# pqpeqr/RL-2048-with-Reinforce-and-Actor-Critic

Hardware: NVIDIA B200
Metric: 2048 env-steps/sec (random-legal batched env stepping, 1M packed boards per GPU) (higher is better)
Workload: dtype u64

## Files before the change

rl-2048-with-reinforce-and-actor-critic_b200/csrc/b2048_device.cuh:

```cuda
#pragma once
#include <stdint.h>

#if defined(__CUDACC__)
#define B2_HD __host__ __device__ __forceinline__
#else
#define B2_HD static inline
#endif

namespace b2 {

struct Board {
    uint32_t lo, hi;
};

B2_HD Board make_board(uint64_t b) { return Board{(uint32_t)b, (uint32_t)(b >> 32)}; }
B2_HD uint64_t to_u64(Board b) { return (uint64_t)b.lo | ((uint64_t)b.hi << 32); }

B2_HD uint32_t prmt(uint32_t x, uint32_t y, uint32_t s) {
#if defined(__CUDA_ARCH__)
    uint32_t r;
    asm("prmt.b32 %0, %1, %2, %3;" : "=r"(r) : "r"(x), "r"(y), "r"(s));
    return r;
#else
    uint64_t v = (uint64_t)x | ((uint64_t)y << 32);
// ... 48 lines not shown
    asm("lop3.b32 %0, %1, %2, %3, 0xE4;" : "=r"(r) : "r"(on1), "r"(on0), "r"(mask));
    return r;
#else
    return (on1 & mask) | (on0 & ~mask);
#endif
}

B2_HD uint32_t nz8(uint32_t x) { return (((x & 0x77777777u) + 0x77777777u) | x) & 0x88888888u; }

struct Rand4 {
    uint32_t w0, w1, w2, w3;
};

B2_HD Rand4 philox4x32_10(uint32_t c0, uint32_t c1, uint32_t c2, uint32_t c3, uint32_t k0, uint32_t k1) {
    const uint32_t M0 = 0xD2511F53u, M1 = 0xCD9E8D57u, W0 = 0x9E3779B9u, W1 = 0xBB67AE85u;
#pragma unroll
    for (int r = 0; r < 10; ++r) {
        uint32_t h0 = mulhi(M0, c0), l0 = M0 * c0;
        uint32_t h1 = mulhi(M1, c2), l1 = M1 * c2;
        c0 = h1 ^ c1 ^ k0;
        c1 = l1;
        c2 = h0 ^ c3 ^ k1;
        c3 = l0;
        k0 += W0;
        k1 += W1;
    }
    return Rand4{c0, c1, c2, c3};
}

struct PhiloxKeys {
    uint32_t k0[10], k1[10];
};
B2_HD PhiloxKeys make_keys(uint64_t seed) {
    PhiloxKeys k;
    uint32_t a = (uint32_t)seed, b = (uint32_t)(seed >> 32);
    for (int r = 0; r < 10; ++r) { k.k0[r] = a; k.k1[r] = b; a += 0x9E3779B9u; b += 0xBB67AE85u; }
    return k;
}
B2_HD Rand4 philox_keyed(uint32_t c0, uint32_t c1, uint32_t c2, uint32_t c3, const PhiloxKeys& k) {
    const uint32_t M0 = 0xD2511F53u, M1 = 0xCD9E8D57u;
#pragma unroll
    for (int r = 0; r < 10; ++r) {
        uint64_t p0 = (uint64_t)M0 * c0, p1 = (uint64_t)M1 * c2;
        c0 = (uint32_t)(p1 >> 32) ^ c1 ^ k.k0[r];
        c1 = (uint32_t)p1;
        c2 = (uint32_t)(p0 >> 32) ^ c3 ^ k.k1[r];
        c3 = (uint32_t)p0;
    }
    return Rand4{c0, c1, c2, c3};
}
B2_HD Rand4 stream_keyed(const PhiloxKeys& k, uint64_t gid, uint32_t t, uint32_t domain) {
    return philox_keyed((uint32_t)gid, (uint32_t)(gid >> 32), t, domain, k);
}

B2_HD Rand4 stream(uint64_t seed, uint64_t gid, uint32_t t, uint32_t domain) {
    return philox4x32_10((uint32_t)gid, (uint32_t)(gid >> 32), t, domain, (uint32_t)seed, (uint32_t)(seed >> 32));
}

struct Xform {
    uint32_t st;
    uint32_t sm;
    uint32_t f_lo, f_hi, i_lo, i_hi;
};

B2_HD Xform xform_for(uint32_t a) {
    const uint64_t F_LO = 0x3210260423016240ull, F_HI = 0x7654371567457351ull;
    const uint64_t I_LO = 0x3210735123016240ull, I_HI = 0x7654624067457351ull;
    uint32_t sh = 16u * a;
    Xform x;
    x.st = (a & 1u) ? 0u : 12u;
    x.sm = ((a ^ (a >> 1)) & 1u) ? 4u : 0u;
    x.f_lo = (uint32_t)(F_LO >> sh);
    x.f_hi = (uint32_t)(F_HI >> sh);
    x.i_lo = (uint32_t)(I_LO >> sh);
    x.i_hi = (uint32_t)(I_HI >> sh);
    return x;
}

B2_HD uint32_t blk_transpose(uint32_t x, uint32_t s) {
    return bitsel(0x0F0F0000u, x << s, bitsel(0x0000F0F0u, x >> s, x));
}
B2_HD uint32_t nib_swap(uint32_t x, uint32_t s) {
    return bitsel(0xF0F0F0F0u, x << s, x >> s);
}

B2_HD Board canon_fwd(Board b, const Xform& x) {
    uint32_t lo = nib_swap(blk_transpose(b.lo, x.st), x.sm);
    uint32_t hi = nib_swap(blk_transpose(b.hi, x.st), x.sm);
    return Board{prmt(lo, hi, x.f_lo), prmt(lo, hi, x.f_hi)};
}
B2_HD Board canon_inv(Board b, const Xform& x) {
    uint32_t lo = prmt(b.lo, b.hi, x.i_lo), hi = prmt(b.lo, b.hi, x.i_hi);
    return Board{blk_transpose(nib_swap(lo, x.sm), x.st), blk_transpose(nib_swap(hi, x.sm), x.st)};
}

B2_HD void row_move_left(uint32_t row, uint32_t& out, uint32_t& merge) {
    uint32_t cells[4];
    int n = 0;
#pragma unroll
    for (int c = 0; c < 4; ++c) {
        uint32_t e = (row >> (4 * c)) & 0xFu;
        if (e) cells[n++] = e;
    }
    out = 0;
    merge = 0;
    int i = 0, w = 0, nm = 0;
    while (i < n) {
        if (i + 1 < n && cells[i] == cells[i + 1]) {
            uint32_t e = cells[i] + 1;
            out |= (e > 15u ? 15u : e) << (4 * w);
            merge |= (e > 15u ? 1u : e) << (4 * nm);
            ++nm;
            i += 2;
        } else {
            out |= cells[i] << (4 * w);
            i += 1;
        }
        ++w;
    }
}

struct MoveResult {
    Board board;
    uint32_t merge;
};

template <typename LutL, typename LutM>
B2_HD MoveResult move_board(Board b, uint32_t a, LutL lut_left, LutM lut_merge) {
    Xform x = xform_for(a);
    Board c = canon_fwd(b, x);
    uint32_t i0 = c.lo & 0xFFFFu, i1 = c.lo >> 16, i2 = c.hi & 0xFFFFu, i3 = c.hi >> 16;
    uint32_t r0 = lut_left[i0], r1 = lut_left[i1], r2 = lut_left[i2], r3 = lut_left[i3];
    uint32_t m0 = lut_merge[i0], m1 = lut_merge[i1], m2 = lut_merge[i2], m3 = lut_merge[i3];
    Board moved{r0 | (r1 << 16), r2 | (r3 << 16)};
    MoveResult res;
    res.board = canon_inv(moved, x);
    res.merge = m0 | (m1 << 8) | (m2 << 16) | (m3 << 24);
    return res;
}

struct MergeStats {
    uint32_t n;
    uint32_t sum_log2;
    uint32_t sum;
    uint32_t max_exp;
    bool overflow;
};

B2_HD MergeStats merge_stats(uint32_t m, bool want_sum, bool want_max) {
    MergeStats s;
    uint32_t nzb = nz8(m);
    s.n = (uint32_t)popc(nzb);
    uint32_t is1 = nzb & ~nz8(m ^ 0x11111111u);
    s.overflow = is1 != 0u;
    uint32_t pairs = (m & 0x0F0F0F0Fu) + ((m >> 4) & 0x0F0F0F0Fu);
    pairs = (pairs & 0x00FF00FFu) + ((pairs >> 8) & 0x00FF00FFu);
    s.sum_log2 = (pairs + (pairs >> 16)) & 0xFFFFu;
    s.sum = 0;
    s.max_exp = 0;
    if (s.overflow) s.sum_log2 += 15u * (uint32_t)popc(is1);
    if (want_sum || want_max) {
#pragma unroll
        for (int k = 0; k < 8; ++k) {
            uint32_t e = (m >> (4 * k)) & 0xFu;
            e = (e == 1u) ? 16u : e;
            if (want_sum) s.sum += e ? (1u << e) : 0u;
// ... 84 lines not shown
```

rl-2048-with-reinforce-and-actor-critic_b200/csrc/b2048_env.cu:

```cuda
#include <cuda_runtime.h>

#include <cstdio>
#include <cstdlib>

#include "b2048_internal.h"
#include "b2048_ptx.cuh"
#include "b2048_step_fast.cuh"

namespace b2 {

__global__ void build_lut_kernel(uint16_t* __restrict__ lut_left, uint8_t* __restrict__ lut_merge) {
    uint32_t row = blockIdx.x * blockDim.x + threadIdx.x;
    if (row >= 65536u) return;
    uint32_t out, merge;
    row_move_left(row, out, merge);
    lut_left[row] = (uint16_t)out;
    lut_merge[row] = (uint8_t)merge;
}

__global__ void build_small_tables_kernel(uint8_t* __restrict__ small) {
    static_assert(B2048_SMALL_BYTES == B2048_TABLES_BYTES - B2048_LUT_BYTES, "small table size mismatch");
    const uint32_t tid = threadIdx.x;
    if (tid < 256u) small_table_entry_agg(tid, reinterpret_cast<AggEntry*>(small + B2048_SMALL_AGG_OFF)[tid]);
    if (tid < 4u) small_table_entry_sel(tid, reinterpret_cast<SelEntry*>(small + B2048_SMALL_SEL_OFF)[tid]);
// ... 159 lines not shown
            if (cfg.action_mode == B2048_ACT_BUFFER) io.action = args.action[i];
            if (args.flags_in) io.mask_in = args.flags_in[i];
        }
        if (!lut_ready) {
            mbar_wait(s_u32(&mbar), 0);
            lut_ready = true;
        }
        bool frozen = false;
        Board board_before = io.board;
        if (args.ep_len && valid) frozen = args.ep_len[i] != 0;
        step_one(io, cfg, opt, args.seed, args.gid0 + (uint64_t)i, args.t, lut_left, lut_merge);
        if (valid && frozen) {
            uint32_t m = legal_mask(board_before);
            uint32_t f = args.flags_in ? (uint32_t)args.flags_in[i]
                                       : (m | ((m == 0u && (board_before.lo | board_before.hi) != 0u) ? B2048_F_DONE : 0u));
            args.board_out[i] = to_u64(board_before);
            if (args.action_out) args.action_out[i] = 0;
            if (args.merge_sum) args.merge_sum[i] = 0;
            if (args.reward) args.reward[i] = 0.0f;
            if (args.reward64) args.reward64[i] = 0.0;
            args.flags[i] = (uint8_t)(f & ~B2048_F_CHANGED);
            io.board = board_before;
        } else if (valid) {
            if (args.ep_len && (io.flags & (B2048_F_DONE | B2048_F_TRUNC))) args.ep_len[i] = (int32_t)args.ep_t;
            args.board_out[i] = to_u64(io.board);
            if (args.score) args.score[i] = io.score;
            if (args.step) args.step[i] = io.step;
            if (args.max_exp) args.max_exp[i] = (uint8_t)io.max_exp;
            if (args.action_out) args.action_out[i] = (uint8_t)io.action_played;
            if (args.merge_sum) args.merge_sum[i] = io.merge_sum;
            if (args.reward) args.reward[i] = (float)io.reward;
            if (args.reward64) args.reward64[i] = io.reward;
            args.flags[i] = (uint8_t)io.flags;
        }
        if (args.obs != nullptr && cfg.obs_mode != B2048_OBS_NONE) {
            const int64_t warp_base = base + (tid & ~31);
            if (cfg.obs_mode == B2048_OBS_ONEHOT) store_obs_onehot(args.obs, io.board, warp_base, args.n, lane);
            else store_obs16(args.obs, io.board, warp_base, args.n, lane, cfg.obs_mode, cfg.obs_log2_scale);
        }
    }
}

template <int kAct, bool kTrack, bool kPlain>
__global__ void __launch_bounds__(1024, 1) step_fast_kernel(const __grid_constant__ StepArgs args) {
    extern __shared__ __align__(128) uint8_t smem[];
    __shared__ uint64_t mbar;
    const int tid = threadIdx.x;
    const bool dbg = args.debug_clock != nullptr && tid == 0 && (blockIdx.x == 0 || blockIdx.x == 147);
    long long* dc = dbg ? args.debug_clock + (blockIdx.x == 0 ? 0 : 16) : nullptr;
    int dci = 0;
    if (dbg) { dc[dci++] = (long long)globaltimer(); dc[dci++] = clock64(); }
    pdl_launch_dependents();
    stage_tables<true>(smem, args, &mbar);
    FastTables T;
    T.left = reinterpret_cast<const uint16_t*>(smem);
    T.merge = smem + B2048_LUT_LEFT_BYTES;
    T.agg = reinterpret_cast<const AggEntry*>(smem + B2048_LUT_BYTES + B2048_SMALL_AGG_OFF);
    T.sel = reinterpret_cast<const SelEntry*>(smem + B2048_LUT_BYTES + B2048_SMALL_SEL_OFF);
    T.act = smem + B2048_LUT_BYTES + B2048_SMALL_ACT_OFF;
    pdl_wait();

    const b2048_env_cfg& cfg = args.cfg;
    if constexpr (kPlain) {
        const uint32_t n = (uint32_t)args.n, stride = gridDim.x * 1024u;
        uint32_t i = blockIdx.x * 1024u + (uint32_t)tid;
        uint2 bw_next = make_uint2(0u, 0u);
        uint32_t act_next = 0u, fin_next = 0u, score_next = 0u, step_next = 0u, max_next = 2u;
        auto request = [&](uint32_t k) {
            bw_next = *reinterpret_cast<const uint2*>(args.board_in + k);
            if (kAct == B2048_ACT_BUFFER) act_next = args.action[k];
            else if (kAct != B2048_ACT_RANDOM_ANY) fin_next = args.flags_in[k];
            if (kTrack) { score_next = args.score[k]; step_next = args.step[k]; max_next = args.max_exp[k]; }
        };
        if (i < n) request(i);
        Rand4 rnd = stream_keyed(args.keys, args.gid0 + (uint64_t)i, args.t, B2048_DOM_STEP);
        mbar_wait(s_u32(&mbar), 0);
        for (; i < n; i += stride) {
            FastIO io;
            io.lo = bw_next.x; io.hi = bw_next.y;
            io.score = score_next; io.step = step_next; io.max_exp = max_next;
            io.action = act_next; io.mask_in = fin_next;
            const uint32_t inext = i + stride;
            if (inext < n) request(inext);
            step_fast_rnd<kAct, kTrack, false>(io, cfg, rnd, args.seed, args.gid0 + (uint64_t)i, args.t, T);
            *reinterpret_cast<uint2*>(args.board_out + i) = make_uint2(io.lo, io.hi);
            if (kTrack) { args.score[i] = io.score; args.step[i] = io.step; args.max_exp[i] = (uint8_t)io.max_exp; }
            args.reward[i] = io.reward;
            args.flags[i] = (uint8_t)io.flags;
            if (inext < n) rnd = stream_keyed(args.keys, args.gid0 + (uint64_t)inext, args.t, B2048_DOM_STEP);
        }
        return;
    }
    bool ready = false;
    const int64_t stride = (int64_t)gridDim.x * 1024;
    int64_t i = (int64_t)blockIdx.x * 1024 + tid;
    uint2 bw_next = make_uint2(0u, 0u);
    uint32_t act_next = 0u, fin_next = 0u;
    if (i < args.n) {
        bw_next = *reinterpret_cast<const uint2*>(args.board_in + i);
        if (kAct == B2048_ACT_BUFFER) act_next = args.action[i];
        if (args.flags_in) fin_next = args.flags_in[i];
    }
    for (; i < args.n; i += stride) {
        FastIO io;
        const uint2 bw = bw_next;
        const uint32_t fin = fin_next;
        io.lo = bw.x; io.hi = bw.y;
        io.score = 0u; io.step = 0u; io.max_exp = 2u; io.mask_in = 0u;
        io.action = act_next;
        const int64_t inext = i + stride;
        if (inext < args.n) {
            bw_next = *reinterpret_cast<const uint2*>(args.board_in + inext);
            if (kAct == B2048_ACT_BUFFER) act_next = args.action[inext];
            if (args.flags_in) fin_next = args.flags_in[inext];
        }
        if (kTrack) { io.score = args.score[i]; io.step = args.step[i]; io.max_exp = args.max_exp[i]; }
        if (kAct == B2048_ACT_RANDOM_LEGAL || kAct == B2048_ACT_PRIORITY)
            io.mask_in = args.flags_in ? fin : legal_mask(Board{io.lo, io.hi});
        bool frozen = false;
        if (args.ep_len) frozen = args.ep_len[i] != 0;
        if (!ready) {
            mbar_wait(s_u32(&mbar), 0);
            ready = true;
            if (dbg) dc[dci++] = clock64();
        }
        if (frozen) {
            uint32_t m = legal_mask(Board{io.lo, io.hi});
            uint32_t f = args.flags_in ? fin : (m | ((m == 0u && (io.lo | io.hi) != 0u) ? B2048_F_DONE : 0u));
            *reinterpret_cast<uint2*>(args.board_out + i) = bw;
            if (args.action_out) args.action_out[i] = 0;
            if (args.merge_sum) args.merge_sum[i] = 0;
            args.reward[i] = 0.0f;
            args.flags[i] = (uint8_t)(f & ~B2048_F_CHANGED);
            continue;
        }
        step_fast<kAct, kTrack>(io, cfg, args.keys, args.seed, args.gid0 + (uint64_t)i, args.t, T);
        if (args.ep_len && (io.flags & (B2048_F_DONE | B2048_F_TRUNC))) args.ep_len[i] = (int32_t)args.ep_t;
        *reinterpret_cast<uint2*>(args.board_out + i) = make_uint2(io.lo, io.hi);
        if (kTrack) { args.score[i] = io.score; args.step[i] = io.step; args.max_exp[i] = (uint8_t)io.max_exp; }
        if (args.action_out) args.action_out[i] = (uint8_t)io.action;
        if (args.merge_sum) args.merge_sum[i] = io.merge_sum;
        args.reward[i] = io.reward;
        args.flags[i] = (uint8_t)io.flags;
        if (dbg && dci < 12) dc[dci++] = clock64();
    }
    if (dbg) { const unsigned long long gt = globaltimer(); dc[14] = clock64(); dc[15] = (long long)gt; }
}

template <int kAct, bool kTrack, bool kPlain>
static cudaError_t launch_fast_one(int grid, size_t smem, cudaStream_t s, const StepArgs& a, bool pdl) {
    cudaLaunchConfig_t lc = {};
    lc.gridDim = dim3((unsigned)grid); lc.blockDim = dim3(1024); lc.dynamicSmemBytes = smem; lc.stream = s;
    cudaLaunchAttribute at[1];
    at[0].id = cudaLaunchAttributeProgrammaticStreamSerialization;
    at[0].val.programmaticStreamSerializationAllowed = 1;
    lc.attrs = at; lc.numAttrs = pdl ? 1u : 0u;
    return cudaLaunchKernelEx(&lc, step_fast_kernel<kAct, kTrack, kPlain>, a);
}
template <int kAct>
static cudaError_t launch_fast(bool track, int grid, size_t smem, cudaStream_t s, const StepArgs& a, bool pdl) {
    const bool plain = a.ep_len == nullptr && a.action_out == nullptr && a.merge_sum == nullptr && a.debug_clock == nullptr &&
                       (kAct == B2048_ACT_BUFFER || kAct == B2048_ACT_RANDOM_ANY || a.flags_in != nullptr) &&
                       a.n < ((int64_t)1 << 31) - (int64_t)grid * 1024 &&
                       !cfg_is_shaped(a.cfg);
    if (plain) return track ? launch_fast_one<kAct, true, true>(grid, smem, s, a, pdl) : launch_fast_one<kAct, false, true>(grid, smem, s, a, pdl);
    return track ? launch_fast_one<kAct, true, false>(grid, smem, s, a, pdl) : launch_fast_one<kAct, false, false>(grid, smem, s, a, pdl);
}
// ... 375 lines not shown
```

rl-2048-with-reinforce-and-actor-critic_b200/csrc/b2048_policy_tc.cu:

```cuda
#include <cuda_bf16.h>
#include <cuda_runtime.h>

#include <cstdio>
#include <cstdlib>

#include "b2048_device.cuh"
#include "b2048_internal.h"
#include "b2048_step_fast.cuh"
#include "b2048_tc.cuh"

namespace b2 {

__global__ void __launch_bounds__(256) policy_tc_prepare_kernel(const float* __restrict__ W1, const float* __restrict__ b1,
                                                                 const float* __restrict__ W2, const float* __restrict__ b2,
                                                                 const float* __restrict__ W3, const float* __restrict__ b3,
                                                                 int n_out, uint8_t* __restrict__ img) {
    const int tid = blockIdx.x * blockDim.x + threadIdx.x;
    const int nth = gridDim.x * blockDim.x;
    auto put = [&](size_t off, float v) { *reinterpret_cast<__nv_bfloat16*>(img + off) = __float2bfloat16_rn(v); };
    for (int idx = tid; idx < TC_H * TC_H; idx += nth) {
        int k = idx / TC_H, n = idx - k * TC_H;
        int slab = k >> 6, kc = (k & 63) >> 3, ke = k & 7;
        put((size_t)IMG_W2 + (size_t)slab * 32768 + (size_t)n * 128 + (size_t)((kc ^ (n & 7)) * 16) + ke * 2, W2[idx]);
    }
// ... 338 lines not shown
                        }
                        if (kRollout) args.ro_actions[slice * stride + b] = (uint8_t)a;
                        else args.action[s] = (uint8_t)a;
                    }
                }
                if (kRollout) {
                    const int g = j & 1, ord = ord_of(j, r);
                    wait_steps_through(g, ord - 1);
                    sAct[g * TC_M + row] = (uint8_t)a;
                    __syncwarp();
                    if (lane == 0) mbar_arrive(bar_act0 + 8u * g);
                    if (dbg) args.debug_clock[8 * item + 6] = clock64();
                    if (!prefetch && item + 1 < n_items) {
                        wait_inputs_of(jn, rn);
                        encode_a1(jn, rn);
                    }
                }
                j = jn; r = rn;
                ph ^= 1u;
            }
        } else if (kRollout) {
            {
                const uint4* src = reinterpret_cast<const uint4*>(args.tables + B2048_LUT_BYTES);
                uint4* dst = reinterpret_cast<uint4*>(smem + SM_TBL);
                for (int i = tid - TC_THREADS; i < B2048_SMALL_BYTES / 16; i += TC_ENV_THREADS) dst[i] = src[i];
                bar_sync(1, TC_ENV_THREADS);
            }
            const int grp = (warp - 21) >> 2;
            const uint32_t bar_act = bar_act0 + 8u * grp, bar_step = bar_step0 + 8u * grp;
            FastTables T;
            T.left = reinterpret_cast<const uint16_t*>(args.tables);
            T.merge = args.tables + B2048_LUT_LEFT_BYTES;
            T.agg = reinterpret_cast<const AggEntry*>(smem + SM_TBL + B2048_SMALL_AGG_OFF);
            T.sel = reinterpret_cast<const SelEntry*>(smem + SM_TBL + B2048_SMALL_SEL_OFF);
            T.act = smem + SM_TBL + B2048_SMALL_ACT_OFF;

            struct EnvIn { uint64_t bd; uint32_t score, step, max_exp, fin; int32_t ep; };
            auto load_in = [&](int j, int r) {
                EnvIn e = {0ull, 0u, 0u, 2u, 0u, 0};
                const int64_t s = tile_of(j) * TC_M + row;
                if (s < n_slots) {
                    const int64_t b = args.slot_map ? args.slot_map[s] : s;
                    const int64_t i = slice_of(r) * args.ro_stride + b;
                    e.bd = args.ro_boards[i]; e.fin = args.ro_flags[i];
                    e.score = args.score[b]; e.step = args.step[b]; e.max_exp = args.max_exp[b];
                    if (args.ep_len) e.ep = args.ep_len[b];
                }
                return e;
            };
            const int own_tiles = (n_owned + 1 - grp) >> 1;
            const int n_rounds = n_owned > 0 ? n_items / n_owned : 0;
            int j = grp, r = own_tiles > 0 ? 0 : n_rounds;
            EnvIn cur = r < n_rounds ? load_in(j, r) : EnvIn{0ull, 0u, 0u, 2u, 0u, 0};
            while (r < n_rounds) {
                int jn = j + 2, rn = r;
                if (jn >= n_owned) { jn = grp; ++rn; }
                const int item = r * n_owned + j;
                const int64_t s = tile_of(j) * TC_M + row;
                const int64_t slice = slice_of(r);
                const bool valid = s < n_slots;
                const int64_t b = (valid && args.slot_map) ? args.slot_map[s] : s;
                const uint32_t t_env = args.t0 + (uint32_t)slice + 1u;
                FastIO io;
                io.lo = (uint32_t)cur.bd; io.hi = (uint32_t)(cur.bd >> 32);
                io.score = cur.score; io.step = cur.step; io.max_exp = cur.max_exp; io.mask_in = 0u;
                const uint32_t fin = cur.fin;
                const bool frozen = cur.ep != 0;
                Rand4 rr = Rand4{0u, 0u, 0u, 0u};
                if (valid && !frozen) rr = stream_keyed(args.keys, args.gid0 + (uint64_t)b, t_env, B2048_DOM_STEP);
                EnvIn nxt = cur;
                if (own_tiles > 1 && rn < n_rounds) nxt = load_in(jn, rn);
                mbar_wait(bar_act, ph);
                const bool dbg = args.debug_clock != nullptr && blockIdx.x == 0 && (tid - TC_THREADS) % TC_ENV_GROUP == 0 && item < 8;
                if (dbg) args.debug_clock[8 * item + 7] = clock64();
                if (valid) {
                    const int64_t o = (slice + 1) * args.ro_stride + b;
                    if (frozen) {
                        args.ro_boards[o] = cur.bd;
                        args.ro_rewards[slice * args.ro_stride + b] = 0.0f;
                        io.flags = fin & ~B2048_F_CHANGED;
                        args.ro_flags[o] = (uint8_t)io.flags;
                    } else {
                        io.action = sAct[grp * TC_M + row];
                        step_fast_rnd<B2048_ACT_BUFFER, true, kShaped>(io, args.cfg, rr, args.seed, args.gid0 + (uint64_t)b, t_env, T);
                        if (args.ep_len && (io.flags & (B2048_F_DONE | B2048_F_TRUNC))) {
                            args.ep_len[b] = (int32_t)(slice + 1);
                            cur.ep = (int32_t)(slice + 1);
                        }
                        args.ro_boards[o] = (uint64_t)io.lo | ((uint64_t)io.hi << 32);
                        args.score[b] = io.score; args.step[b] = io.step; args.max_exp[b] = (uint8_t)io.max_exp;
                        args.ro_rewards[slice * args.ro_stride + b] = io.reward;
                        args.ro_flags[o] = (uint8_t)io.flags;
                    }
                }
                if (own_tiles == 1) {
                    nxt.bd = (uint64_t)io.lo | ((uint64_t)io.hi << 32);
                    nxt.score = io.score; nxt.step = io.step; nxt.max_exp = io.max_exp; nxt.fin = io.flags; nxt.ep = cur.ep;
                }
                cur = nxt;
                j = jn; r = rn;
                __threadfence_block();
                __syncwarp();
                if (lane == 0) mbar_arrive(bar_step);
                ph ^= 1u;
            }
        }
    }

    tmem_teardown(warp == 16, tmem_base, 512u);
}

void launch_tc_prepare(const b2048_mlp_desc* mlp, uint8_t* img, cudaStream_t stream) {
    policy_tc_prepare_kernel<<<64, 256, 0, stream>>>(mlp->W[0], mlp->b[0], mlp->W[1], mlp->b[1], mlp->W[2], mlp->b[2],
                                                      mlp->dims[3], img);
}

int ensure_tc_image(b2048_handle* h) {
    if (!h->tc_image) {
        cudaError_t e = cudaMalloc(&h->tc_image, IMG_BYTES);
        if (e != cudaSuccess) return check_cuda(e, "cudaMalloc(tc_image)");
    }
    if (!(h->attrs & ATTR_POLICY_TC)) {
        cudaError_t e = cudaFuncSetAttribute(policy_tc_kernel<false>, cudaFuncAttributeMaxDynamicSharedMemorySize, SM_TOTAL2);
        if (e != cudaSuccess) return check_cuda(e, "cudaFuncSetAttribute(policy_tc_kernel)");
        e = cudaFuncSetAttribute(policy_tc_kernel<true, false>, cudaFuncAttributeMaxDynamicSharedMemorySize, SM_TOTAL_RO);
        if (e != cudaSuccess) return check_cuda(e, "cudaFuncSetAttribute(policy_tc_kernel<rollout>)");
        e = cudaFuncSetAttribute(policy_tc_kernel<true, true>, cudaFuncAttributeMaxDynamicSharedMemorySize, SM_TOTAL_RO);
        if (e != cudaSuccess) return check_cuda(e, "cudaFuncSetAttribute(policy_tc_kernel<rollout, shaped>)");
        h->attrs |= ATTR_POLICY_TC;
    }
    return B2048_OK;
}

static int print_debug_clock(const b2048_handle* h, cudaStream_t stream) {
    long long hbuf[96];
    { int st = debug_clock_read(h, hbuf, 96, stream); if (st != B2048_OK) return st; }
    for (int k = 0; k < 6; ++k)
        fprintf(stderr,
                "[tc clock] item %d: wait_d1+d3 %lld epi1 %lld wait_d2 %lld epi2 %lld | total %lld | to next %lld | io: d3 seen +%lld, "
                "sample %lld | env: actions seen +%lld\n",
                k, hbuf[8 * k + 1] - hbuf[8 * k], hbuf[8 * k + 2] - hbuf[8 * k + 1], hbuf[8 * k + 3] - hbuf[8 * k + 2],
                hbuf[8 * k + 4] - hbuf[8 * k + 3], hbuf[8 * k + 4] - hbuf[8 * k], hbuf[8 * k + 8] - hbuf[8 * k],
                hbuf[8 * k + 5] - hbuf[8 * k], hbuf[8 * k + 6] - hbuf[8 * k + 5], hbuf[8 * k + 7] - hbuf[8 * k]);
    for (int k = 0; k < 4; ++k)
        fprintf(stderr, "[tc clock] item %d: mma: layer 2 starts +%lld, last H2 slab seen +%lld, d3 committed +%lld | sampler waits for d3 from +%lld\n",
                k, hbuf[64 + 4 * k] - hbuf[8 * k], hbuf[64 + 4 * k + 1] - hbuf[8 * k], hbuf[64 + 4 * k + 2] - hbuf[8 * k],
                hbuf[64 + 4 * k + 3] - hbuf[8 * k]);
    for (int k = 0; k < 4; ++k) fprintf(stderr, "[tc clock] item %d: slowest epilogue warp leaves epilogue 2 at +%lld\n", k, hbuf[80 + k] - hbuf[8 * k]);
    return B2048_OK;
}

int launch_policy_tc(b2048_handle* h, const b2048_mlp_desc* mlp, const uint64_t* board, const uint8_t* mask_flags,
                     uint8_t* action, float* probs, float* logits, int64_t n, uint64_t seed, uint64_t gid0, uint32_t t,
                     int greedy, cudaStream_t stream, bool rebuild_image) {
    if (!fixed_tc_net(mlp) || mlp->dims[3] != 4 || h->smem_optin < SM_TOTAL2) return B2048_ERR_UNSUPPORTED;
    { int st = ensure_tc_image(h); if (st != B2048_OK) return st; }
    if (rebuild_image) launch_tc_prepare(mlp, h->tc_image, stream);
    PolicyTcArgs a{};
    a.img = h->tc_image; a.board = board; a.mask_flags = mask_flags; a.action = action; a.probs = probs; a.logits = logits;
    a.n_out = 4; a.n = n; a.keys = make_keys(seed); a.gid0 = gid0; a.t = t; a.greedy = greedy; a.obs_mode = mlp->obs_mode;
    a.obs_scale = mlp->obs_log2_scale; a.seed = seed; a.n_steps = 1; a.ro_stride = n;
    a.debug_clock = debug_clock_begin(h, B2048_DBG_TC_CLOCKS, stream);
    int64_t tiles = (n + TC_M - 1) / TC_M;
    int grid = (int)(tiles < h->num_sms ? tiles : h->num_sms);
    policy_tc_kernel<false><<<grid, TC_THREADS, SM_TOTAL2, stream>>>(a);
    int st = check_cuda(cudaGetLastError(), "policy_tc_kernel launch");
    if (st == B2048_OK && a.debug_clock) st = print_debug_clock(h, stream);
// ... 50 lines not shown
```

rl-2048-with-reinforce-and-actor-critic_b200/csrc/b2048_step_fast.cuh:

```cuda
#pragma once
#include "b2048_step.cuh"

namespace b2 {

struct SelEntry {
    uint32_t f_lo, f_hi, i_lo, i_hi;
    uint32_t st, sm, pad0, pad1;
};
struct AggEntry {
    uint32_t agg;
    uint32_t orm;
};
#define B2048_SMALL_AGG_OFF 0
#define B2048_SMALL_SEL_OFF 2048
#define B2048_SMALL_ACT_OFF (2048 + 128)
#define B2048_SMALL_BYTES (2048 + 128 + 64)

B2_HD void small_table_entry_agg(uint32_t byte, AggEntry& e) {
    e.agg = 0; e.orm = 0;
    for (int k = 0; k < 2; ++k) {
        uint32_t m = (byte >> (4 * k)) & 0xFu;
        if (!m) continue;
        uint32_t ex = m == 1u ? 16u : m;
        e.agg += (1u << ex) + (ex << 20) + (1u << 28);
        e.orm |= 1u << ex;
    }
}
B2_HD void small_table_entry_sel(uint32_t a, SelEntry& s) {
    Xform x = xform_for(a);
    s.f_lo = x.f_lo & 0xFFFFu; s.f_hi = x.f_hi & 0xFFFFu; s.i_lo = x.i_lo & 0xFFFFu; s.i_hi = x.i_hi & 0xFFFFu;
    s.st = x.st; s.sm = x.sm; s.pad0 = 0; s.pad1 = 0;
}
B2_HD uint32_t small_table_entry_act(uint32_t mask, uint32_t j) {
    uint32_t m = mask;
    for (uint32_t q = 0; q < j; ++q) m &= m - 1;
    return m ? (uint32_t)ffs0(m) : 0u;
}

struct FastTables {
    const uint16_t* left;
    const uint8_t* merge;
    const AggEntry* agg;
    const SelEntry* sel;
    const uint8_t* act;
};

struct FastIO {
    uint32_t lo, hi;
    uint32_t score, step, max_exp;
    uint32_t action;
    uint32_t mask_in;
    float reward;
    uint32_t flags;
    int32_t merge_sum;
};

template <int kAct, bool kTrack, bool kShaped = true>
B2_HD void step_fast_rnd(FastIO& io, const b2048_env_cfg& cfg, const Rand4& rnd, uint64_t seed, uint64_t gid, uint32_t t,
                         const FastTables& T) {

    uint32_t a;
    if (kAct == B2048_ACT_BUFFER) a = io.action & 3u;
    else if (kAct == B2048_ACT_RANDOM_ANY) a = rnd.w2 >> 30;
    else if (kAct == B2048_ACT_PRIORITY) a = pick_priority(io.mask_in & 0xFu, (uint32_t)cfg.action_priority);
    else {
        uint32_t m4 = io.mask_in & 0xFu;
        a = T.act[m4 * 4u + mulhi(rnd.w2, (uint32_t)popc(m4))];
    }
    io.action = a;

    const SelEntry s = T.sel[a];
    uint32_t clo = nib_swap(blk_transpose(io.lo, s.st), s.sm), chi = nib_swap(blk_transpose(io.hi, s.st), s.sm);
    uint32_t flo = prmt(clo, chi, s.f_lo), fhi = prmt(clo, chi, s.f_hi);
    uint32_t i0 = flo & 0xFFFFu, i1 = shr_fma<16>(flo), i2 = fhi & 0xFFFFu, i3 = shr_fma<16>(fhi);
    uint32_t r0 = T.left[i0], r1 = T.left[i1], r2 = T.left[i2], r3 = T.left[i3];
    const AggEntry g0 = T.agg[T.merge[i0]], g1 = T.agg[T.merge[i1]], g2 = T.agg[T.merge[i2]], g3 = T.agg[T.merge[i3]];
    uint32_t agg = g0.agg + g1.agg + g2.agg + g3.agg;
    uint32_t orm = g0.orm | g1.orm | g2.orm | g3.orm;
    uint32_t mlo = r0 + (r1 << 16), mhi = r2 + (r3 << 16);
    uint32_t plo = prmt(mlo, mhi, s.i_lo), phi = prmt(mlo, mhi, s.i_hi);
    uint32_t vlo = blk_transpose(nib_swap(plo, s.sm), s.st), vhi = blk_transpose(nib_swap(phi, s.sm), s.st);
    const bool changed = ((vlo ^ io.lo) | (vhi ^ io.hi)) != 0u;

    const uint32_t msum = agg & 0xFFFFFu;
    io.merge_sum = (int32_t)msum;
    if (kTrack) {
        io.score += msum;
        io.step += 1u;
    }

    const uint32_t nb_lo = shr_fma<3>(nz8(vlo)), nb_hi = shr_fma<3>(nz8(vhi));
    const uint32_t zb_lo = nb_lo ^ 0x11111111u, zb_hi = nb_hi ^ 0x11111111u;
    const uint32_t P_lo = zb_lo * 0x11111111u, P_hi = zb_hi * 0x11111111u;
    const uint32_t c_lo = shr_fma<28>(P_lo), c_hi = shr_fma<28>(P_hi);
    const uint32_t n_empty = c_lo + c_hi;
    uint32_t k = mulhi(rnd.w0, n_empty);
    const bool in_hi = k >= c_lo;
    const uint32_t P = in_hi ? P_hi : P_lo;
    k = in_hi ? k - c_lo : k;
    const uint32_t addk = (0x7Fu - k) * 0x01010101u;
    const uint32_t Ge = ((P & 0x0F0F0F0Fu) + addk) & 0x80808080u;
    const uint32_t Go = ((shr_fma<4>(P) & 0x0F0F0F0Fu) + addk) & 0x80808080u;
    const uint32_t G = shr_fma<7>(Ge) | shr_fma<3>(Go);
    const uint32_t iso = G & (0u - G);
    uint32_t val = rnd.w1 >= 0xE6666667u ? 2u : 1u;
    val = (changed && n_empty != 0u) ? val : 0u;
    const uint32_t ins = iso * val;
    const uint32_t hsel = in_hi ? 0xFFFFFFFFu : 0u;
    uint32_t nlo = vlo | (ins & ~hsel), nhi = vhi | (ins & hsel);
    const uint32_t spawned = val ? iso : 0u;

    const uint32_t N = (nb_lo | (spawned & ~hsel)) | ((nb_hi | (spawned & hsel)) << 1);
    const uint32_t MH = 0x03330333u, MV = 0x11113333u;
    const uint32_t Nr = shr_fma<4>(N);
    const uint32_t EH = shr_fma<3>(nz8(nlo ^ shr_fma<4>(nlo))) | shr_fma<2>(nz8(nhi ^ shr_fma<4>(nhi)));
    const uint32_t hmerge = ~EH & N & MH;
    const uint32_t left = (~N & Nr & MH) | hmerge;
    const uint32_t right = (N & ~Nr & MH) | hmerge;
    const uint32_t Nd = (shr_fma<16>(N) & 0x00003333u) | ((N * 32768u) & 0x11110000u);
    const uint32_t EV = shr_fma<3>(nz8(nlo ^ funnel_r(nlo, nhi, 16))) | shr_fma<2>(nz8(nhi ^ shr_fma<16>(nhi)));
    const uint32_t vmerge = ~EV & N & MV;
    const uint32_t up = (~N & Nd & MV) | vmerge;
    const uint32_t down = (N & ~Nd & MV) | vmerge;
    uint32_t mask = (up ? 1u : 0u) | (right ? 2u : 0u) | (down ? 4u : 0u) | (left ? 8u : 0u);
    const bool done = (mask == 0u) & ((nlo | nhi) != 0u);

    uint32_t max_merged = 31u - (uint32_t)
#if defined(__CUDA_ARCH__)
        __clz((int)(orm | 1u));
#else
        __builtin_clz(orm | 1u);
#endif
    const uint32_t base = cfg.reward_mode == B2048_REWARD_SUM ? msum : (shr_fma<20>(agg) & 0xFFu);
    double r = dmul((double)base, cfg.base_reward_scale);
    if (kShaped && cfg.empty_tile_reward != 0.0) r = dadd(r, dmul(cfg.empty_tile_reward, (double)(n_empty - (val ? 1u : 0u))));
    if (kShaped && cfg.merge_reward != 0.0) r = dadd(r, dmul(cfg.merge_reward, (double)(agg >> 28)));
    if (kTrack && max_merged >= 3u && max_merged > io.max_exp) {
        io.max_exp = max_merged;
        if (kShaped && cfg.bonus_mode != B2048_BONUS_OFF) {
            const double bonus = cfg.bonus_mode == B2048_BONUS_RAW ? (double)(1u << max_merged) : (double)max_merged;
            r = dadd(r, dmul(bonus, cfg.bonus_scale));
        }
    }
    r = dadd(r, cfg.step_reward);
    if (kShaped && done && cfg.endgame_penalty != 0.0) r = dadd(r, cfg.endgame_penalty);
    io.reward = (float)r;

    bool trunc = false;
    if (kTrack) trunc = cfg.max_steps > 0 && io.step >= (uint32_t)cfg.max_steps && !done;
    uint32_t f = (changed ? B2048_F_CHANGED : 0u) | (done ? B2048_F_DONE : 0u) | (trunc ? B2048_F_TRUNC : 0u) |
                 ((orm >> 16) & 1u ? B2048_F_OVERFLOW : 0u);
    if (cfg.auto_reset && (done | trunc)) {
        Board nbd = reset_board(seed, gid, t);
        nlo = nbd.lo; nhi = nbd.hi;
        if (kTrack) { io.score = 0u; io.step = 0u; io.max_exp = 2u; }
        mask = legal_mask(nbd);
    }
    io.lo = nlo; io.hi = nhi;
    io.flags = f | mask;
}

template <int kAct, bool kTrack, bool kShaped = true>
B2_HD void step_fast(FastIO& io, const b2048_env_cfg& cfg, const PhiloxKeys& keys, uint64_t seed, uint64_t gid,
                     uint32_t t, const FastTables& T) {
    step_fast_rnd<kAct, kTrack, kShaped>(io, cfg, stream_keyed(keys, gid, t, B2048_DOM_STEP), seed, gid, t, T);
}
inline bool cfg_is_shaped(const b2048_env_cfg& c) {
    return c.empty_tile_reward != 0.0 || c.merge_reward != 0.0 || c.endgame_penalty != 0.0 || c.bonus_mode != B2048_BONUS_OFF;
}

}
```

Measured before the change: 58.86 billion.

## Use multiply-based symmetry transforms and precomputed reset-board table in step kernel

Replaces the variable-shift symmetry transforms with mask- and multiply-based variants whose per-action parameters come from the selector table, so the shifts run on the FMA pipe instead of the ALU pipe. Replaces the auto-reset path, which rebuilt the start board and recomputed its legal mask, with a lookup into a constexpr 1024-entry constant-memory table indexed by keyed random words. This cuts ALU instructions in the hot loop and in the reset branch. In exchange, constant-memory reads with divergent indices serialize within a warp, and the reset distribution must match the old reset_board semantics. A SASS pipe-counting script is also added.

```diff
diff --git a/profiles/sass_pipes.py b/profiles/sass_pipes.py
--- /dev/null
+++ b/profiles/sass_pipes.py
@@ -0,0 +1,97 @@
+#!/usr/bin/env python
+import collections, os, re, subprocess, sys
+
+ROOT = os.path.dirname(os.path.dirname(os.path.abspath(__file__)))
+DEFAULT_LIB = os.path.join(ROOT, "rl-2048-with-reinforce-and-actor-critic_b200", "libb2048.so")
+DEFAULT_KERNELS = ["_ZN2b216step_fast_kernelILi3ELb1ELb1EEEvNS_8StepArgsE"]
+
+ALU = {"LOP3", "LOP", "SHF", "SHL", "SHR", "SEL", "FSEL", "ISETP", "FSETP", "IADD3", "IADD", "VIADD", "VIADDMNMX", "LEA",
+       "PRMT", "POPC", "FLO", "BREV", "IMNMX", "VIMNMX", "IABS", "BMSK", "SGXT", "PLOP3", "P2R", "R2P", "MOV", "ICMP",
+       "ISCADD", "CS2R"}
+FMA = {"IMAD", "FFMA", "FMUL", "FADD", "HFMA2", "HADD2", "HMUL2", "IDP", "IMUL"}
+FP64 = {"DADD", "DMUL", "DFMA", "DSETP", "F2F", "F2I", "I2F", "I2FP", "F2FP"}
+MEM = {"LDS", "LDG", "STG", "STS", "LD", "ST", "ATOM", "ATOMS", "RED", "REDG", "LDC", "LDL", "STL"}
+PIPES = ["alu", "fma", "fp64/conv", "mem", "ctrl", "uniform", "other"]
+
+LINE = re.compile(r"\s*/\*([0-9a-f]{4,})\*/\s+(@!?U?P[T0-9]+\s+)?([A-Z0-9_]+)((?:\.[A-Z0-9_]+)*)\s*([^;]*);")
+
+
+def pipe(op):
+    if op in ALU:
+        return "alu"
+    if op in FMA:
+        return "fma"
+    if op in FP64:
+        return "fp64/conv"
+    if op in MEM:
+        return "mem"
+    if op in {"BRA", "BSSY", "BSYNC", "EXIT", "NOP", "WARPSYNC", "YIELD", "BAR", "PREEXIT", "CALL", "RET", "BPT"}:
+        return "ctrl"
+    if op.startswith("U") or op in {"S2UR", "R2UR", "S2R", "CS2R"}:
+        return "uniform"
+    return "other"
+
+
+def sass_of(path, kernel):
+    out = subprocess.run(["cuobjdump", "-sass", "-fun", kernel, path], capture_output=True, text=True)
+    if out.returncode != 0 or "Function" not in out.stdout:
+        sys.exit(f"cuobjdump found no function {kernel} in {path}:\n{out.stderr}")
+    ins = []
+    for line in out.stdout.splitlines():
+        m = LINE.match(line)
+        if m:
+            ins.append((int(m.group(1), 16), m.group(3), m.group(3) + m.group(4), m.group(5), bool(m.group(2))))
+    return ins
+
+
+def regions(ins):
+    idx = {a[0]: k for k, a in enumerate(ins)}
+    best = None
+    for a, op, full, arg, pred in ins:
+        if op == "BRA" and pred:
+            m = re.search(r"0x([0-9a-f]+)", arg)
+            tgt = int(m.group(1), 16) if m else None
+            if tgt is not None and tgt < a and tgt in idx and (best is None or a - tgt > best[1] - best[0]):
+                best = (tgt, a)
+    if best is None:
+        sys.exit("no loop found")
+    lo, hi = idx[best[0]], idx[best[1]]
+    first_st = next((k for k in range(lo, hi + 1) if ins[k][1] in ("STG", "ST")), hi + 1)
+    blocks = []
+    for k in range(lo, first_st):
+        a, op, full, arg, pred = ins[k]
+        if op == "BSSY":
+            m = re.search(r"(B\d+),\s*0x([0-9a-f]+)", arg)
+            end = int(m.group(2), 16)
+            if end in idx and idx[end] <= first_st:
+                blocks.append((k, idx[end]))
+    reset = max(blocks, key=lambda b: b[1] - b[0], default=None)
+    in_reset = set(range(reset[0], reset[1] + 1)) if reset else set()
+    return {"main": [ins[k] for k in range(lo, first_st) if k not in in_reset],
+            "reset": [ins[k] for k in sorted(in_reset)],
+            "tail": [ins[k] for k in range(first_st, hi + 1)]}
+
+
+def main():
+    args = [a for a in sys.argv[1:] if a != "-v"]
+    verbose = "-v" in sys.argv[1:]
+    path = args[0] if args else DEFAULT_LIB
+    kernels = args[1:] or DEFAULT_KERNELS
+    for kern in kernels:
+        regs = regions(sass_of(path, kern))
+        print(f"{kern}")
+        print(f"{'region':8s} {'instrs':>6s} " + " ".join(f"{p:>9s}" for p in PIPES))
+        tot = collections.Counter()
+        for name, body in regs.items():
+            c = collections.Counter(pipe(x[1]) for x in body)
+            tot.update(c)
+            print(f"{name:8s} {len(body):6d} " + " ".join(f"{c[p]:9d}" for p in PIPES))
+        print(f"{'loop':8s} {sum(tot.values()):6d} " + " ".join(f"{tot[p]:9d}" for p in PIPES))
+        if verbose:
+            for name, body in regs.items():
+                c = collections.Counter(x[2] for x in body)
+                print(f"  {name}: " + ", ".join(f"{k} {v}" for k, v in c.most_common()))
+
+
+if __name__ == "__main__":
+    main()
diff --git a/rl-2048-with-reinforce-and-actor-critic_b200/csrc/b2048_device.cuh b/rl-2048-with-reinforce-and-actor-critic_b200/csrc/b2048_device.cuh
--- a/rl-2048-with-reinforce-and-actor-critic_b200/csrc/b2048_device.cuh
+++ b/rl-2048-with-reinforce-and-actor-critic_b200/csrc/b2048_device.cuh
@@ -154,6 +154,12 @@
 }
 B2_HD uint32_t nib_swap(uint32_t x, uint32_t s) {
     return bitsel(0xF0F0F0F0u, x << s, x >> s);
+}
+B2_HD uint32_t blk_transpose_m(uint32_t x, uint32_t tm) {
+    return bitsel(tm, x * 4096u, bitsel(shr_fma<12>(tm), shr_fma<12>(x), x));
+}
+B2_HD uint32_t nib_swap_m(uint32_t x, uint32_t nl, uint32_t nr) {
+    return bitsel(0xF0F0F0F0u, x * nl, shr_fma<4>(x * nr));
 }
 
 B2_HD Board canon_fwd(Board b, const Xform& x) {
diff --git a/rl-2048-with-reinforce-and-actor-critic_b200/csrc/b2048_env.cu b/rl-2048-with-reinforce-and-actor-critic_b200/csrc/b2048_env.cu
--- a/rl-2048-with-reinforce-and-actor-critic_b200/csrc/b2048_env.cu
+++ b/rl-2048-with-reinforce-and-actor-critic_b200/csrc/b2048_env.cu
@@ -265,7 +265,7 @@
             io.action = act_next; io.mask_in = fin_next;
             const uint32_t inext = i + stride;
             if (inext < n) request(inext);
-            step_fast_rnd<kAct, kTrack, false>(io, cfg, rnd, args.seed, args.gid0 + (uint64_t)i, args.t, T);
+            step_fast_rnd<kAct, kTrack, false>(io, cfg, rnd, args.keys, args.gid0 + (uint64_t)i, args.t, T);
             *reinterpret_cast<uint2*>(args.board_out + i) = make_uint2(io.lo, io.hi);
             if (kTrack) { args.score[i] = io.score; args.step[i] = io.step; args.max_exp[i] = (uint8_t)io.max_exp; }
             args.reward[i] = io.reward;
diff --git a/rl-2048-with-reinforce-and-actor-critic_b200/csrc/b2048_policy_tc.cu b/rl-2048-with-reinforce-and-actor-critic_b200/csrc/b2048_policy_tc.cu
--- a/rl-2048-with-reinforce-and-actor-critic_b200/csrc/b2048_policy_tc.cu
+++ b/rl-2048-with-reinforce-and-actor-critic_b200/csrc/b2048_policy_tc.cu
@@ -444,7 +444,7 @@
                         args.ro_flags[o] = (uint8_t)io.flags;
                     } else {
                         io.action = sAct[grp * TC_M + row];
-                        step_fast_rnd<B2048_ACT_BUFFER, true, kShaped>(io, args.cfg, rr, args.seed, args.gid0 + (uint64_t)b, t_env, T);
+                        step_fast_rnd<B2048_ACT_BUFFER, true, kShaped>(io, args.cfg, rr, args.keys, args.gid0 + (uint64_t)b, t_env, T);
                         if (args.ep_len && (io.flags & (B2048_F_DONE | B2048_F_TRUNC))) {
                             args.ep_len[b] = (int32_t)(slice + 1);
                             cur.ep = (int32_t)(slice + 1);
diff --git a/rl-2048-with-reinforce-and-actor-critic_b200/csrc/b2048_step_fast.cuh b/rl-2048-with-reinforce-and-actor-critic_b200/csrc/b2048_step_fast.cuh
--- a/rl-2048-with-reinforce-and-actor-critic_b200/csrc/b2048_step_fast.cuh
+++ b/rl-2048-with-reinforce-and-actor-critic_b200/csrc/b2048_step_fast.cuh
@@ -5,7 +5,7 @@
 
 struct SelEntry {
     uint32_t f_lo, f_hi, i_lo, i_hi;
-    uint32_t st, sm, pad0, pad1;
+    uint32_t tm, nl, nr, pad;
 };
 struct AggEntry {
     uint32_t agg;
@@ -29,12 +29,63 @@
 B2_HD void small_table_entry_sel(uint32_t a, SelEntry& s) {
     Xform x = xform_for(a);
     s.f_lo = x.f_lo & 0xFFFFu; s.f_hi = x.f_hi & 0xFFFFu; s.i_lo = x.i_lo & 0xFFFFu; s.i_hi = x.i_hi & 0xFFFFu;
-    s.st = x.st; s.sm = x.sm; s.pad0 = 0; s.pad1 = 0;
+    s.tm = x.st ? 0x0F0F0000u : 0u;
+    s.nl = x.sm ? 16u : 1u;
+    s.nr = x.sm ? 1u : 16u;
+    s.pad = 0;
 }
 B2_HD uint32_t small_table_entry_act(uint32_t mask, uint32_t j) {
     uint32_t m = mask;
     for (uint32_t q = 0; q < j; ++q) m &= m - 1;
     return m ? (uint32_t)ffs0(m) : 0u;
+}
+
+struct StartTables {
+    Board board[1024];
+    uint8_t mask[1024];
+};
+constexpr uint32_t cells_legal_mask(const uint8_t (&e)[16]) {
+    const int dr[4] = {-1, 0, 1, 0}, dc[4] = {0, 1, 0, -1};
+    uint32_t m = 0;
+    for (int c = 0; c < 16; ++c)
+        for (int a = 0; a < 4; ++a) {
+            const int r2 = c / 4 + dr[a], c2 = c % 4 + dc[a];
+            if (e[c] && r2 >= 0 && r2 < 4 && c2 >= 0 && c2 < 4 && (e[4 * r2 + c2] == 0 || e[4 * r2 + c2] == e[c])) m |= 1u << a;
+        }
+    return m;
+}
+constexpr StartTables make_start_tables() {
+    StartTables s{};
+    for (uint32_t c1 = 0; c1 < 16; ++c1)
+        for (uint32_t k2 = 0; k2 < 16; ++k2) {
+            const uint32_t c2 = (k2 + (k2 >= c1 ? 1u : 0u)) & 15u;
+            for (uint32_t v = 0; v < 4; ++v) {
+                uint8_t e[16] = {};
+                e[c2] = (uint8_t)(1 + (v & 1));
+                e[c1] = (uint8_t)(1 + (v >> 1));
+                uint64_t b = 0;
+                for (int c = 0; c < 16; ++c) b |= (uint64_t)e[c] << (4 * c);
+                s.board[(c1 * 16 + k2) * 4 + v] = Board{(uint32_t)b, (uint32_t)(b >> 32)};
+                s.mask[(c1 * 16 + k2) * 4 + v] = (uint8_t)cells_legal_mask(e);
+            }
+        }
+    return s;
+}
+#if defined(__CUDACC__)
+static __constant__ StartTables g_start_tables_dev = make_start_tables();
+#endif
+static constexpr StartTables g_start_tables_host = make_start_tables();
+
+B2_HD Board start_board(const Rand4& w, uint32_t& mask) {
+#if defined(__CUDA_ARCH__)
+    const StartTables& S = g_start_tables_dev;
+#else
+    const StartTables& S = g_start_tables_host;
+#endif
+    const uint32_t i = (mulhi(w.w0, 16u) * 16u + mulhi(w.w2, 15u)) * 4u + (w.w1 >= 0xE6666667u ? 2u : 0u) +
+                       (w.w3 >= 0xE6666667u ? 1u : 0u);
+    mask = S.mask[i];
+    return S.board[i];
 }
 
 struct FastTables {
@@ -56,8 +107,8 @@
 };
 
 template <int kAct, bool kTrack, bool kShaped = true>
-B2_HD void step_fast_rnd(FastIO& io, const b2048_env_cfg& cfg, const Rand4& rnd, uint64_t seed, uint64_t gid, uint32_t t,
-                         const FastTables& T) {
+B2_HD void step_fast_rnd(FastIO& io, const b2048_env_cfg& cfg, const Rand4& rnd, const PhiloxKeys& keys, uint64_t gid,
+                         uint32_t t, const FastTables& T) {
 
     uint32_t a;
     if (kAct == B2048_ACT_BUFFER) a = io.action & 3u;
@@ -70,7 +121,7 @@
     io.action = a;
 
     const SelEntry s = T.sel[a];
-    uint32_t clo = nib_swap(blk_transpose(io.lo, s.st), s.sm), chi = nib_swap(blk_transpose(io.hi, s.st), s.sm);
+    uint32_t clo = nib_swap_m(blk_transpose_m(io.lo, s.tm), s.nl, s.nr), chi = nib_swap_m(blk_transpose_m(io.hi, s.tm), s.nl, s.nr);
     uint32_t flo = prmt(clo, chi, s.f_lo), fhi = prmt(clo, chi, s.f_hi);
     uint32_t i0 = flo & 0xFFFFu, i1 = shr_fma<16>(flo), i2 = fhi & 0xFFFFu, i3 = shr_fma<16>(fhi);
     uint32_t r0 = T.left[i0], r1 = T.left[i1], r2 = T.left[i2], r3 = T.left[i3];
@@ -79,7 +130,7 @@
     uint32_t orm = g0.orm | g1.orm | g2.orm | g3.orm;
     uint32_t mlo = r0 + (r1 << 16), mhi = r2 + (r3 << 16);
     uint32_t plo = prmt(mlo, mhi, s.i_lo), phi = prmt(mlo, mhi, s.i_hi);
-    uint32_t vlo = blk_transpose(nib_swap(plo, s.sm), s.st), vhi = blk_transpose(nib_swap(phi, s.sm), s.st);
+    uint32_t vlo = blk_transpose_m(nib_swap_m(plo, s.nl, s.nr), s.tm), vhi = blk_transpose_m(nib_swap_m(phi, s.nl, s.nr), s.tm);
     const bool changed = ((vlo ^ io.lo) | (vhi ^ io.hi)) != 0u;
 
     const uint32_t msum = agg & 0xFFFFFu;
@@ -151,19 +202,18 @@
     uint32_t f = (changed ? B2048_F_CHANGED : 0u) | (done ? B2048_F_DONE : 0u) | (trunc ? B2048_F_TRUNC : 0u) |
                  ((orm >> 16) & 1u ? B2048_F_OVERFLOW : 0u);
     if (cfg.auto_reset && (done | trunc)) {
-        Board nbd = reset_board(seed, gid, t);
+        const Board nbd = start_board(stream_keyed(keys, gid, t, B2048_DOM_RESET), mask);
         nlo = nbd.lo; nhi = nbd.hi;
         if (kTrack) { io.score = 0u; io.step = 0u; io.max_exp = 2u; }
-        mask = legal_mask(nbd);
     }
     io.lo = nlo; io.hi = nhi;
     io.flags = f | mask;
 }
 
 template <int kAct, bool kTrack, bool kShaped = true>
-B2_HD void step_fast(FastIO& io, const b2048_env_cfg& cfg, const PhiloxKeys& keys, uint64_t seed, uint64_t gid,
-                     uint32_t t, const FastTables& T) {
-    step_fast_rnd<kAct, kTrack, kShaped>(io, cfg, stream_keyed(keys, gid, t, B2048_DOM_STEP), seed, gid, t, T);
+B2_HD void step_fast(FastIO& io, const b2048_env_cfg& cfg, const PhiloxKeys& keys, uint64_t ,
+                     uint64_t gid, uint32_t t, const FastTables& T) {
+    step_fast_rnd<kAct, kTrack, kShaped>(io, cfg, stream_keyed(keys, gid, t, B2048_DOM_STEP), keys, gid, t, T);
 }
 inline bool cfg_is_shaped(const b2048_env_cfg& c) {
     return c.empty_tile_reward != 0.0 || c.merge_reward != 0.0 || c.endgame_penalty != 0.0 || c.bonus_mode != B2048_BONUS_OFF;
```

After: 61.32 billion, median of 6. +4.2%, better.
